# simonhmartin/genomics_general

Hardware: AMD Instinct MI355X
Metric: windows_per_sec (higher is better)
Workload: dtype u32 bit-planes / int32 counts / f64 statistics

## Files before the change

### genomics_general_amd/csrc/pg_pair2.hip

```cpp
#include "pg_internal.h"
#include "pg_pair_common.h"

#include <algorithm>
#include <cstdlib>
#include <cstring>

typedef __attribute__((address_space(4))) const uint32_t CU32;

__device__ __forceinline__ void store16(uint32_t *p, uint32_t a, uint32_t b, uint32_t c, uint32_t d) {
    *reinterpret_cast<uint4 *>(p) = make_uint4(a, b, c, d);
}

__device__ __forceinline__ void btrans4(uint32_t t0, uint32_t t1, uint32_t t2, uint32_t t3, uint32_t r[4]) {
    const uint32_t lo01 = __builtin_amdgcn_perm(t1, t0, 0x05010400u), hi01 = __builtin_amdgcn_perm(t1, t0, 0x07030602u);
    const uint32_t lo23 = __builtin_amdgcn_perm(t3, t2, 0x05010400u), hi23 = __builtin_amdgcn_perm(t3, t2, 0x07030602u);
    r[0] = __builtin_amdgcn_perm(lo23, lo01, 0x05040100u);
    r[1] = __builtin_amdgcn_perm(lo23, lo01, 0x07060302u);
    r[2] = __builtin_amdgcn_perm(hi23, hi01, 0x05040100u);
    r[3] = __builtin_amdgcn_perm(hi23, hi01, 0x07060302u);
}

struct RowOff { int v[16]; };

__device__ __forceinline__ RowOff make_row_off(int RS) {
    RowOff ro;
#pragma unroll
    for (int s = 0; s < 16; ++s) {
        int t = s * RS;
        asm volatile("" : "+s"(t));
        ro.v[s] = t;
    }
    return ro;
}

__device__ __forceinline__ void word_load(__amdgpu_buffer_rsrc_t rsrc, int b0, int RS, int row0, const RowOff &ro, uint32_t d[32]) {
    const int v0 = b0 + row0 * RS, v1 = v0 + 16 * RS;
#pragma unroll
    for (int s = 0; s < 16; ++s) d[s] = (uint32_t)__builtin_amdgcn_raw_buffer_load_b32(rsrc, v0, ro.v[s], 0);
#pragma unroll
    for (int s = 0; s < 16; ++s) d[16 + s] = (uint32_t)__builtin_amdgcn_raw_buffer_load_b32(rsrc, v1, ro.v[s], 0);
}

__device__ __forceinline__ void word_load16(__amdgpu_buffer_rsrc_t rsrc, int b0, int RS, int row0, const RowOff &ro, uint32_t d[32]) {
    const int v0 = b0 + row0 * RS, v1 = v0 + 16 * RS;
#pragma unroll
    for (int s = 0; s < 16; ++s) d[s] = (uint32_t)__builtin_amdgcn_raw_buffer_load_b16(rsrc, v0, ro.v[s], 0);
#pragma unroll
    for (int s = 0; s < 16; ++s) d[16 + s] = (uint32_t)__builtin_amdgcn_raw_buffer_load_b16(rsrc, v1, ro.v[s], 0);
}

__device__ __forceinline__ uint32_t merge16(uint32_t x0, uint32_t x1) { return pg_nib_expand4(x0) | (pg_nib_expand4(x1) << 4); }

__device__ __forceinline__ void word_called_presence(const uint32_t d[32], uint32_t v[4], uint32_t pa[4]) {
#pragma unroll
    for (int q = 0; q < 4; ++q) {
        const uint32_t *e = d + 8 * q;
        uint32_t r[4];
        btrans4(merge16(e[0], e[1]), merge16(e[2], e[3]), merge16(e[4], e[5]), merge16(e[6], e[7]), r);
        const uint32_t o = r[0] | r[1] | r[2] | r[3];
#pragma unroll
        for (int a = 0; a < 4; ++a) {
            const uint32_t piece = (a >= q ? (o >> (a - q)) : (o << (q - a))) & (0x11111111u << q);
            pa[a] = q ? (pa[a] | piece) : piece;
        }
#pragma unroll
        for (int k = 0; k < 4; ++k) {
            const uint32_t u = r[k] | (r[k] >> 1);
            const uint32_t c = (u | (u >> 2)) & 0x11111111u;
            v[k] = q ? (v[k] | (c << q)) : c;
        }
    }
}

__device__ __forceinline__ void poly_word(__amdgpu_buffer_rsrc_t rsrc, int h0, int RS, uint32_t vlist, const uint32_t SA[3],
                                          const uint32_t SE[2], uint32_t x[PG_XV_PLANES][4]) {
    uint32_t al[4][4];
#pragma unroll
    for (int q = 0; q < 4; ++q) {
        uint32_t d[8];
#pragma unroll
        for (int s = 0; s < 8; ++s) {
            const int row = __builtin_amdgcn_readlane((int)vlist, q * 8 + s) & 0xffff;
            d[s] = (uint32_t)__builtin_amdgcn_raw_buffer_load_b16(rsrc, h0 >> 1, row * RS, 0);
        }
        uint32_t r[4];
        btrans4(merge16(d[0], d[1]), merge16(d[2], d[3]), merge16(d[4], d[5]), merge16(d[6], d[7]), r);
#pragma unroll
        for (int k = 0; k < 4; ++k)
#pragma unroll
            for (int a = 0; a < 4; ++a) {
                const uint32_t piece = (a >= q ? (r[k] >> (a - q)) : (r[k] << (q - a))) & (0x11111111u << q);
                al[a][k] = q ? (al[a][k] | piece) : piece;
            }
    }
#pragma unroll
    for (int k = 0; k < 4; ++k) {
        const uint32_t ex = (al[0][k] & SE[0]) | (al[1][k] & SE[1]);
        x[0][k] = (al[0][k] & SA[0]) | (al[1][k] & SA[1]) | (al[2][k] & SA[2]);
        x[1][k] = (al[0][k] | al[1][k] | al[2][k] | al[3][k]) & ~ex;
    }
}

__device__ __forceinline__ void wave_or4(uint32_t v[4]) {
#define PG_DPP_OR4(ctrl, rmask)                                                                           \
    _Pragma("unroll") for (int i = 0; i < 4; ++i)                                                          \
        v[i] |= (uint32_t)__builtin_amdgcn_update_dpp(0, (int)v[i], ctrl, rmask, 0xf, false)
    PG_DPP_OR4(0x111, 0xf);
    PG_DPP_OR4(0x112, 0xf);
    PG_DPP_OR4(0x114, 0xf);
    PG_DPP_OR4(0x118, 0xf);
    PG_DPP_OR4(0x142, 0xa);
    PG_DPP_OR4(0x143, 0xc);
#undef PG_DPP_OR4
#pragma unroll
    for (int i = 0; i < 4; ++i) v[i] = (uint32_t)__builtin_amdgcn_readlane((int)v[i], 63);
}

__device__ __forceinline__ uint32_t poly_mask(const uint32_t p[4]) {
    return (p[0] & p[1]) | (p[2] & p[3]) | ((p[0] ^ p[1]) & (p[2] ^ p[3]));
}

__device__ __forceinline__ uint32_t tri_mask(const uint32_t p[4]) {
    return (p[0] & p[1] & (p[2] | p[3])) | (p[2] & p[3] & (p[0] | p[1]));
}
__device__ __forceinline__ uint32_t quad_mask(const uint32_t p[4]) { return p[0] & p[1] & p[2] & p[3]; }

__device__ __forceinline__ __amdgpu_buffer_rsrc_t group_rsrc(const int8_t *gt, int RS, int64_t first_row, int nrows) {
    return __builtin_amdgcn_make_buffer_rsrc(const_cast<int8_t *>(gt + first_row * (int64_t)RS), 0, nrows * RS, 0x00020000);
}

template <int NWAVE>
__device__ __forceinline__ bool xv_leader() { return (NWAVE == 1 ? threadIdx.x & 63 : threadIdx.x) == 0; }

struct XvWin {
    uint32_t *xv_base;
    int NP, h0, capw;
    int32_t *nwb, *mismatch;
    bool has_data;

    template <int NWAVE>
    __device__ __forceinline__ bool holds(int slot) const {
        if (slot >= capw) {
            if (xv_leader<NWAVE>()) atomicOr(mismatch, 2);
            return false;
        }
        return has_data;
    }
    __device__ __forceinline__ uint32_t *word(int slot) const { return xv_base + (size_t)slot * PG_XV_PLANES * (size_t)NP + 2 * h0; }
};

__device__ __forceinline__ XvWin make_xv_win(uint32_t *XV, const int64_t *goff, int b, int capg, int NP, int h0, int32_t *nw,
                                             int32_t *mismatch, bool has_data) {
    return {XV + (size_t)goff[b] * capg * PG_XV_PLANES * (size_t)NP, NP, h0, (int)(goff[b + 1] - goff[b]) * capg, &nw[b], mismatch, has_data};
}

template <int NWAVE>
__device__ __forceinline__ int xv_reserve(int32_t *nwb, int n, int *sh_slot) {
    if (NWAVE == 1) {
        int s0 = 0;
        if (xv_leader<1>()) s0 = atomicAdd(nwb, n);
        return __builtin_amdgcn_readfirstlane(s0);
    }
    if (xv_leader<NWAVE>()) *sh_slot = atomicAdd(nwb, n);
    __syncthreads();
    const int slot = __builtin_amdgcn_readfirstlane(*sh_slot);
    __syncthreads();
    return slot;
}

template <int NWAVE>
__device__ __forceinline__ void block_or4(uint32_t pr[4], uint32_t (*sh_pres)[NWAVE][4], int &parity, int lane) {
    wave_or4(pr);
    if (NWAVE > 1) {
        if (lane == 0) {
#pragma unroll
            for (int a = 0; a < 4; ++a) sh_pres[parity][threadIdx.x >> 6][a] = pr[a];
        }
        __syncthreads();
#pragma unroll
        for (int a = 0; a < 4; ++a) {
            uint32_t x = 0u;
#pragma unroll
            for (int wv = 0; wv < NWAVE; ++wv) x |= sh_pres[parity][wv][a];
            pr[a] = __builtin_amdgcn_readfirstlane(x);
        }
        parity ^= 1;
    }
}

__global__ __launch_bounds__(256) void k_presence(const int8_t *__restrict__ gt, int RS, const int64_t *__restrict__ win_lo,
                                                  const int64_t *__restrict__ win_hi, const int64_t *__restrict__ goff,
                                                  uint32_t *__restrict__ pres, int grp) {
    const int b = blockIdx.y, g = blockIdx.x;
    const int64_t lo = win_lo[b], hi = win_hi[b];
    const int W = (int)((hi - lo + 31) >> 5);
    const int w_begin = g * grp;
    if (w_begin >= W) return;
    const int w_end = (w_begin + grp < W) ? w_begin + grp : W;
    const int h0 = 4 * (blockIdx.z * 256 + threadIdx.x);
    const int64_t first = lo + 32ll * w_begin;
    const int nrows = (int)((hi - first) < 32ll * grp ? (hi - first) : 32ll * grp);
    const __amdgpu_buffer_rsrc_t rsrc = group_rsrc(gt, RS, first, nrows);
    uint32_t *dst = pres + (size_t)(goff[b] + g) * grp * 4u;
    const RowOff ro = make_row_off(RS);
    for (int w = w_begin; w < w_end; ++w) {
        uint32_t v[4], pa[4] = {0u, 0u, 0u, 0u};
        if (h0 < 2 * RS) {
            uint32_t d[32];
            word_load16(rsrc, h0 >> 1, RS, (w - w_begin) * 32, ro, d);
            word_called_presence(d, v, pa);
        }
        wave_or4(pa);
#pragma unroll
        for (int a = 0; a < 4; ++a)
            if ((threadIdx.x & 63) == 0 && pa[a]) atomicOr(&dst[(size_t)(w - w_begin) * 4u + a], pa[a]);
    }
}

__global__ __launch_bounds__(256) void k_word_scan(const int64_t *__restrict__ win_lo, const int64_t *__restrict__ win_hi,
                                                   const int64_t *__restrict__ goff, const uint32_t *__restrict__ pres,
                                                   int32_t *__restrict__ nw, int grp) {
    __shared__ int sh[256];
    __shared__ int carry;
    const int b = blockIdx.x, n_win = gridDim.x;
    const int64_t lo = win_lo[b], hi = win_hi[b];
    const int W = (int)((hi - lo + 31) >> 5);
    const int G = (W + grp - 1) / grp;
    if (threadIdx.x == 0) carry = 0;
    __syncthreads();
    for (int g0 = 0; g0 < G; g0 += 256) {
        const int g = g0 + threadIdx.x;
        int words = 0;
        if (g < G) {
            const int nwords = (W - g * grp < grp) ? W - g * grp : grp;
            const uint32_t *src = pres + (size_t)(goff[b] + g) * grp * 4u;
            int cnt = 0;
            for (int w = 0; w < nwords; ++w) {
                const uint32_t p[4] = {src[4 * w], src[4 * w + 1], src[4 * w + 2], src[4 * w + 3]};
                cnt += __builtin_popcount(poly_mask(p)) + __builtin_popcount(tri_mask(p)) + __builtin_popcount(quad_mask(p));
            }
            words = (cnt + 31) >> 5;
        }
        sh[threadIdx.x] = words;
        __syncthreads();
        for (int d = 1; d < 256; d <<= 1) {
            const int v = threadIdx.x >= d ? sh[threadIdx.x - d] : 0;
            __syncthreads();
            sh[threadIdx.x] += v;
            __syncthreads();
        }
        if (g < G) nw[n_win + goff[b] + g] = carry + sh[threadIdx.x] - words;
        __syncthreads();
        if (threadIdx.x == 255) carry += sh[255];
        __syncthreads();
    }
    if (threadIdx.x == 0) nw[b] = carry;
}

template <int TPB, int DIP, int PRES>
__global__ __launch_bounds__(TPB) void k_pack2(const int8_t *__restrict__ gt, int RS, const int64_t *__restrict__ win_lo,
                                               const int64_t *__restrict__ win_hi, const int64_t *__restrict__ goff,
                                               const int64_t *__restrict__ vgoff, uint32_t *__restrict__ Vp, int NPv,
                                               uint32_t *__restrict__ XV, int NP, int32_t *__restrict__ nw,
                                               int32_t *__restrict__ mismatch, const uint32_t *__restrict__ pres, int capg, int grp) {
    constexpr int NWAVE = TPB / 64;
    __shared__ uint32_t sh_pres[2][NWAVE][4];
    __shared__ uint4 sh_gp[PRES ? 1 : PG_GROUP_MAX];
    __shared__ int sh_slot;
    const int b = blockIdx.y, g = blockIdx.x, n_win = gridDim.y;
    const int64_t lo = win_lo[b], hi = win_hi[b];
    const int W = (int)((hi - lo + 31) >> 5);
    const int w_begin = g * grp;
    if (w_begin >= W) return;
    const int w_end = (w_begin + grp < W) ? w_begin + grp : W;
    const int t = blockIdx.z * TPB + threadIdx.x;
    const int lane = threadIdx.x & 63;
    const int h0 = 4 * t;
    const bool has_data = h0 < 2 * RS;
    const int u0 = DIP ? 2 * t : h0;
    const int64_t first = lo + 32ll * w_begin;
    const int nrows = (int)((hi - first) < 32ll * grp ? (hi - first) : 32ll * grp);
    const __amdgpu_buffer_rsrc_t rsrc = group_rsrc(gt, RS, first, nrows);
    uint32_t vlist = (uint32_t)nrows;
    int cnt = 0, nflush = 0, parity = 0;
    uint32_t bad = 0u;
    const XvWin xw = make_xv_win(XV, goff, b, capg, NP, h0, nw, mismatch, has_data);
    const uint32_t *pres_g = pres + (size_t)(goff[b] + g) * grp * 4u;
    const int64_t vg_base = vgoff[b] + (int64_t)(w_begin >> 2);
    const int gbase = PRES ? nw[n_win + goff[b] + g] : 0;
    auto flush = [&]() {
        const int slot = PRES ? gbase + nflush : xv_reserve<NWAVE>(xw.nwb, 1, &sh_slot);
        uint32_t A = 0u, E = 0u;
        {
            const int row = (int)(vlist & 0xffffu), ord = (int)(vlist >> 16);
            if (row < nrows) {
                const int wi = row >> 5, st = row & 31, bit = 4 * (st & 7) + (st >> 3);
                const uint4 pp = PRES ? *reinterpret_cast<const uint4 *>(pres_g + 4 * wi) : sh_gp[PRES ? 0 : wi];
                const uint32_t P = ((pp.x >> bit) & 1u) | (((pp.y >> bit) & 1u) << 1) | (((pp.z >> bit) & 1u) << 2) |
                                   (((pp.w >> bit) & 1u) << 3);
                const uint32_t A0 = P & (0u - P), P1 = P ^ A0, A1 = P1 & (0u - P1), P2 = P1 ^ A1, A2 = P2 & (0u - P2);
                A = ord == 0 ? A0 : (ord == 1 ? A1 : A2);
                E = (A - 1u) & P;
            }
        }
        const int src = (lane & 3) * 8 + ((lane >> 2) & 7);
        A = (uint32_t)__shfl((int)A, src, 64);
        E = (uint32_t)__shfl((int)E, src, 64);
        const uint32_t SA[3] = {(uint32_t)__builtin_amdgcn_ballot_w64(A == 1u), (uint32_t)__builtin_amdgcn_ballot_w64(A == 2u),
                                (uint32_t)__builtin_amdgcn_ballot_w64(A == 4u)};
        const uint32_t SE[2] = {(uint32_t)__builtin_amdgcn_ballot_w64((E & 1u) != 0u),
                                (uint32_t)__builtin_amdgcn_ballot_w64((E & 2u) != 0u)};
        if (xw.holds<NWAVE>(slot)) {
            uint32_t x[PG_XV_PLANES][4];
            poly_word(rsrc, h0, RS, vlist, SA, SE, x);
            uint32_t *o = xw.word(slot);
            store16(o, x[0][0], x[1][0], x[0][1], x[1][1]);
            store16(o + 4, x[0][2], x[1][2], x[0][3], x[1][3]);
        }
        ++nflush;
    };
    uint32_t dn[32];
#pragma unroll
    for (int s = 0; s < 32; ++s) dn[s] = 0u;
    const RowOff ro = make_row_off(RS);
    if (has_data) word_load16(rsrc, h0 >> 1, RS, 0, ro, dn);
    for (int wq = 0; 4 * wq + w_begin < w_end; ++wq) {
        uint32_t vhold[4][4];
#pragma unroll
        for (int k4 = 0; k4 < 4; ++k4) {
            const int w = w_begin + 4 * wq + k4;
            uint32_t v[4] = {0u, 0u, 0u, 0u}, pa[4] = {0u, 0u, 0u, 0u};
            const bool live = w < w_end;
            uint32_t d[32];
#pragma unroll
            for (int s = 0; s < 32; ++s) d[s] = dn[s];
            if (has_data) word_load16(rsrc, h0 >> 1, RS, (w + 1 - w_begin) * 32, ro, dn);
            if (live && has_data) word_called_presence(d, v, pa);
#pragma unroll
            for (int k = 0; k < 4; ++k) vhold[k][k4] = v[k];
            if (DIP) bad |= (v[0] ^ v[1]) | (v[2] ^ v[3]);
            if (live) {
                uint32_t pr[4];
                if (PRES) {
                    const uint32_t *src = pres + ((size_t)(goff[b] + g) * grp + (size_t)(w - w_begin)) * 4u;
#pragma unroll
                    for (int a = 0; a < 4; ++a) pr[a] = __builtin_amdgcn_readfirstlane(src[a]);
                } else {
#pragma unroll
                    for (int a = 0; a < 4; ++a) pr[a] = pa[a];
                    block_or4<NWAVE>(pr, sh_pres, parity, lane);
                }
                if (!PRES && threadIdx.x == 0) sh_gp[PRES ? 0 : w - w_begin] = make_uint4(pr[0], pr[1], pr[2], pr[3]);
                const int row_w = (w - w_begin) * 32;
                const uint32_t m3 = tri_mask(pr);
#pragma unroll 1
                for (int pass = 0; pass < 3; ++pass) {
                    uint32_t m = pass == 0 ? poly_mask(pr) : (pass == 1 ? m3 : quad_mask(pr));
                    if (pass && !m3) break;
                    const uint32_t tag = (uint32_t)pass << 16;
                    while (m) {
                        const int bit = __builtin_ctz(m);
                        m &= m - 1u;
                        vlist = lane == cnt ? ((uint32_t)(row_w + (bit & 3) * 8 + (bit >> 2)) | tag) : vlist;
                        ++cnt;
                    }
                    if (cnt >= 32) {
                        flush();
                        const uint32_t up = (uint32_t)__shfl((int)vlist, (lane + 32) & 63, 64);
                        vlist = lane < 32 ? up : (uint32_t)nrows;
                        cnt -= 32;
                    }
                }
            }
        }
        if (has_data) {
            if (DIP) {
                uint32_t *o = Vp + ((size_t)(vg_base + wq) * NPv + u0) * 4u;
                store16(o, vhold[0][0], vhold[0][1], vhold[0][2], vhold[0][3]);
                store16(o + 4, vhold[2][0], vhold[2][1], vhold[2][2], vhold[2][3]);
            } else {
                uint32_t *o = Vp + ((size_t)(vg_base + wq) * NPv + u0) * 4u;
#pragma unroll
                for (int k = 0; k < 4; ++k)
                    store16(o + 4 * k, vhold[k][0], vhold[k][1], vhold[k][2], vhold[k][3]);
            }
        }
    }
    if (cnt) flush();
    if (DIP && bad) atomicOr(mismatch, 1);
}

__device__ __forceinline__ uint32_t bfi_f0(uint32_t hi, uint32_t lo) { return (hi & 0xF0F0F0F0u) | (lo & 0x0F0F0F0Fu); }

__device__ __forceinline__ void trans_even(const uint32_t e[8], uint32_t r[4]) {
    btrans4(bfi_f0(e[1] << 4, e[0]), bfi_f0(e[3] << 4, e[2]), bfi_f0(e[5] << 4, e[4]), bfi_f0(e[7] << 4, e[6]), r);
}
__device__ __forceinline__ void trans_odd(const uint32_t e[8], uint32_t r[4]) {
    btrans4(bfi_f0(e[1], e[0] >> 4), bfi_f0(e[3], e[2] >> 4), bfi_f0(e[5], e[4] >> 4), bfi_f0(e[7], e[6] >> 4), r);
}
__device__ __forceinline__ void keep_presence(int q, const uint32_t re[4], const uint32_t ro[4], uint32_t Rq[8], uint32_t pa[4]) {
#pragma unroll
    for (int k = 0; k < 4; ++k) {
        Rq[2 * k] = re[k];
        Rq[2 * k + 1] = ro[k];
    }
    const uint32_t o = (re[0] | re[1] | re[2] | re[3]) | (ro[0] | ro[1] | ro[2] | ro[3]);
#pragma unroll
    for (int a = 0; a < 4; ++a) {
        const uint32_t piece = (a >= q ? (o >> (a - q)) : (o << (q - a))) & (0x11111111u << q);
        pa[a] = q ? (pa[a] | piece) : piece;
    }
}

__device__ __forceinline__ void word_called_presence_keep(const uint32_t d[32], uint32_t v[8], uint32_t pa[4], uint32_t R[4][8]) {
#pragma unroll
    for (int q = 0; q < 4; ++q) {
        uint32_t re[4], ro[4];
        trans_even(d + 8 * q, re);
        trans_odd(d + 8 * q, ro);
        keep_presence(q, re, ro, R[q], pa);
#pragma unroll
        for (int k = 0; k < 8; ++k) {
            const uint32_t t = R[q][k] + 0x77777777u;
            const uint32_t c = (q == 3 ? t : (t >> (3 - q))) & (0x11111111u << q);
            v[k] = q ? (v[k] | c) : c;
        }
    }
}

template <int NWAVE, bool STAGED>
struct XvSink {
    XvWin win;
    int *sh_slot;
    uint4 *cell;
    int stride, burst;
    int nxs;

    __device__ __forceinline__ XvSink(const XvWin &w, int *sh_slot_, uint4 *cell_, int stride_, int burst_)
        : win(w), sh_slot(sh_slot_), cell(cell_), stride(stride_), burst(burst_), nxs(0) {}
    __device__ __forceinline__ void flush() {
        if (!nxs) return;
        const int slot0 = xv_reserve<NWAVE>(win.nwb, nxs, sh_slot);
        for (int k = 0; k < nxs; ++k)
            if (win.template holds<NWAVE>(slot0 + k)) {
                uint4 *o = reinterpret_cast<uint4 *>(win.word(slot0 + k));
#pragma unroll
                for (int i = 0; i < 4; ++i) o[i] = cell[(4 * k + i) * stride];
            }
        nxs = 0;
    }
    __device__ __forceinline__ void put(const uint32_t xo[8], const uint32_t vo[8]) {
        if (STAGED) {
            if (win.has_data) {
#pragma unroll
                for (int i = 0; i < 4; ++i) cell[(4 * nxs + i) * stride] = make_uint4(xo[2 * i], vo[2 * i], xo[2 * i + 1], vo[2 * i + 1]);
            }
            if (++nxs == burst) flush();
        } else {
            const int slot = xv_reserve<NWAVE>(win.nwb, 1, sh_slot);
            if (win.template holds<NWAVE>(slot)) {
                uint32_t *o = win.word(slot);
#pragma unroll
                for (int i = 0; i < 4; ++i) store16(o + 4 * i, xo[2 * i], vo[2 * i], xo[2 * i + 1], vo[2 * i + 1]);
            }
        }
    }
};

__device__ __forceinline__ uint32_t nz_nibbles(uint32_t x) { return ((x + 0x77777777u) >> 3) & 0x11111111u; }


template <class Sink>
struct VsCompactor {
    uint32_t cur[8], xo[8], vo[8];
    int cnt;
    uint32_t MA, ME;
    Sink &out;

    __device__ __forceinline__ explicit VsCompactor(Sink &s) : cnt(0), MA(0u), ME(0u), out(s) {
#pragma unroll
        for (int k = 0; k < 8; ++k) cur[k] = xo[k] = vo[k] = 0u;
    }
    __device__ __forceinline__ void finish_dword(int qd) {
        const uint32_t nME = ~ME;
#pragma unroll
        for (int k = 0; k < 8; ++k) {
            xo[k] |= nz_nibbles(cur[k] & MA) << qd;
            vo[k] |= nz_nibbles(cur[k] & nME) << qd;
            cur[k] = 0u;
        }
        MA = 0u;
        ME = 0u;
    }
    __device__ __forceinline__ void store_word() {
        out.put(xo, vo);
#pragma unroll
        for (int k = 0; k < 8; ++k) xo[k] = vo[k] = 0u;
    }
    __device__ __forceinline__ void append(const uint32_t (&Rq)[8], int j, uint32_t A, uint32_t E) {
        const int sh = 4 * (cnt & 7);
#pragma unroll
        for (int k = 0; k < 8; ++k) cur[k] |= __builtin_amdgcn_ubfe(Rq[k], 4 * j, 4) << sh;
        MA |= A << sh;
        ME |= E << sh;
        ++cnt;
        if ((cnt & 7) == 0) {
            finish_dword((cnt >> 3) - 1);
            if (cnt == 32) {
                store_word();
                cnt = 0;
            }
        }
    }
    __device__ __forceinline__ void finish() {
        if (cnt & 7) finish_dword(cnt >> 3);
        if (cnt) store_word();
    }
};

template <class Sink>
__device__ __forceinline__ void emit_poly_sites(const uint32_t pr[4], const uint32_t (&R)[4][8], VsCompactor<Sink> &vs, int lane) {
    const uint32_t m0 = poly_mask(pr);
    if (m0) {
        const int lb = lane & 31;
        const uint32_t Pl = __builtin_amdgcn_ubfe(pr[0], lb, 1) | (__builtin_amdgcn_ubfe(pr[1], lb, 1) << 1) |
                            (__builtin_amdgcn_ubfe(pr[2], lb, 1) << 2) | (__builtin_amdgcn_ubfe(pr[3], lb, 1) << 3);
        const uint32_t A0l = Pl & (0u - Pl);
#pragma unroll
        for (int q = 0; q < 4; ++q) {
            uint32_t mq = m0 & (0x11111111u << q);
            while (mq) {
                const int bit = __builtin_ctz(mq);
                mq &= mq - 1u;
                vs.append(R[q], bit >> 2, (uint32_t)__builtin_amdgcn_readlane((int)A0l, bit), 0u);
            }
        }
        const uint32_t m3 = tri_mask(pr);
        if (m3) {
#pragma unroll 1
            for (int pass = 1; pass < 3; ++pass) {
                uint32_t m = pass == 1 ? m3 : quad_mask(pr);
                while (m) {
                    const int bit = __builtin_ctz(m);
                    m &= m - 1u;
                    const uint32_t P = (uint32_t)__builtin_amdgcn_readlane((int)Pl, bit);
                    const uint32_t A0 = P & (0u - P), P1 = P ^ A0, A1 = P1 & (0u - P1), P2 = P1 ^ A1, A2 = P2 & (0u - P2);
                    const uint32_t A = pass == 1 ? A1 : A2;
                    const int q = bit & 3;
                    if (q == 0) vs.append(R[0], bit >> 2, A, (A - 1u) & P);
                    else if (q == 1) vs.append(R[1], bit >> 2, A, (A - 1u) & P);
                    else if (q == 2) vs.append(R[2], bit >> 2, A, (A - 1u) & P);
                    else vs.append(R[3], bit >> 2, A, (A - 1u) & P);
                }
            }
        }
    }
}

constexpr int PACK_FUSE_XC = 2;
constexpr int PACK_FUSE_NB = 3;
constexpr int PACK_FUSE_SPINS = 1 << 22;

__device__ __forceinline__ void fuse_frags(const uint4 *fb, int s, int UW, const int ia[4], const int ib[2], v8i fa_[4], v8i fb_[2]) {
#pragma unroll
    for (int p = 0; p < 4; ++p) {
        const uint4 x = fb[2 * s * UW + ia[p]];
        fa_[p][0] = (int)x.x; fa_[p][1] = (int)x.y; fa_[p][2] = (int)x.z; fa_[p][3] = (int)x.w;
    }
#pragma unroll
    for (int p = 0; p < 2; ++p) {
        const uint4 x = fb[2 * s * UW + ib[p]];
        fb_[p][0] = (int)x.x; fb_[p][1] = (int)x.y; fb_[p][2] = (int)x.z; fb_[p][3] = (int)x.w;
    }
}

template <int DIP>
__device__ __forceinline__ void pack3_fused(const int8_t *__restrict__ gt, int RS, const int64_t *__restrict__ win_lo,
                                            const int64_t *__restrict__ win_hi, const int64_t *__restrict__ goff,
                                            uint32_t *__restrict__ XV, int NP, int32_t *__restrict__ nw,
                                            int32_t *__restrict__ mismatch, int capg, const PgFuseArgs &fa) {
    constexpr int VN = DIP ? 4 : 8;
    extern __shared__ uint4 fz_lds[];
    int b, kp;
    if (!pg_deal_window(blockIdx.x, fa.kparts, fa.n_win, b, kp)) return;
    const int UW = 32 * fa.T;
    const int lane = threadIdx.x & 63, wave = __builtin_amdgcn_readfirstlane(threadIdx.x >> 6);
    uint4 *const frag = fz_lds;
    uint4 *const stage_x = fz_lds + PACK_FUSE_NB * 8 * UW + wave * (PACK_FUSE_XC * 4 * 64);
    int *const ready = reinterpret_cast<int *>(fz_lds + PACK_FUSE_NB * 8 * UW + 8 * (PACK_FUSE_XC * 4 * 64)), *const done = ready + PACK_FUSE_NB;
    const int64_t lo = win_lo[b], hi = win_hi[b];
    const int W = (int)((hi - lo + 31) >> 5);
    const int w_begin = (int)((long long)W * kp / fa.kparts), w_end = (int)((long long)W * (kp + 1) / fa.kparts);
    const int nit = (w_end - w_begin + 7) >> 3;
    const int h0 = 8 * lane;
    const bool has_data = h0 < 2 * RS;
    const int u0 = VN * lane;
    uint32_t bad = 0u;
    typedef XvSink<1, true> Sink;
    Sink xs(make_xv_win(XV, goff, b, capg, NP, h0, nw, mismatch, has_data), nullptr,  stage_x + lane,  64,
             PACK_FUSE_XC);
    VsCompactor<Sink> vs(xs);
    auto word_rsrc = [&](int w) -> __amdgpu_buffer_rsrc_t {
        const int64_t row = lo + 32ll * w;
        const int n = w < w_end ? (int)((hi - row) < 32 ? (hi - row) : 32) : 0;
        return group_rsrc(gt, RS, n ? row : lo, n);
    };
    const int r = lane & 31, kb = lane >> 5;
    int ia[4], ib[2];
#pragma unroll
    for (int p = 0; p < 4; ++p) ia[p] = kb * UW + 32 * (int)fa.a[wave][p] + r;
#pragma unroll
    for (int p = 0; p < 2; ++p) ib[p] = kb * UW + 32 * (int)fa.b[wave][p] + r;
    v16f acc[4];
#pragma unroll
    for (int p = 0; p < 4; ++p)
#pragma unroll
        for (int e = 0; e < 16; ++e) acc[p][e] = 0.0f;
    if (threadIdx.x < 2 * PACK_FUSE_NB) ready[threadIdx.x] = threadIdx.x == 2 * PACK_FUSE_NB - 1 ? -8 : 0;
    for (int i = threadIdx.x; i < 8 * UW; i += 512) frag[(PACK_FUSE_NB - 1) * 8 * UW + i] = make_uint4(0u, 0u, 0u, 0u);
    bool stalled = false;
    auto wait_ge = [&](int *ctr, int target) {
        for (int spins = 0; __builtin_amdgcn_readfirstlane(__hip_atomic_load(ctr, __ATOMIC_ACQUIRE, __HIP_MEMORY_SCOPE_WORKGROUP)) < target;) {
            __builtin_amdgcn_s_sleep(1);
            if (++spins > PACK_FUSE_SPINS) { stalled = true; break; }
        }
    };
    auto arrive = [&](int *ctr) {
        if (lane == 0) __hip_atomic_fetch_add(ctr, 1, __ATOMIC_RELEASE, __HIP_MEMORY_SCOPE_WORKGROUP);
    };
    uint32_t dn[32];
#pragma unroll
    for (int s = 0; s < 32; ++s) dn[s] = 0u;
    const RowOff ro = make_row_off(RS);
    const int lane_off = has_data ? 4 * lane : 0x40000000;
    word_load(word_rsrc(w_begin + wave), lane_off, RS, 0, ro, dn);
    __syncthreads();
    int slot = 0, round8 = 0, pslot = PACK_FUSE_NB - 1, pround8 = -8;
    for (int it = 0; it < nit; ++it) {
        const int w = w_begin + 8 * it + wave;
        uint32_t pa[4] = {0u, 0u, 0u, 0u};
        uint32_t R[4][8];
        const bool live = w < w_end;
        uint32_t d[32];
#pragma unroll
        for (int s = 0; s < 32; ++s) d[s] = dn[s];
        word_load(word_rsrc(w + 8), lane_off, RS, 0, ro, dn);
        wait_ge(&ready[pslot], pround8 + 8);
        const uint4 *fb = frag + pslot * 8 * UW;
#pragma unroll
        for (int q = 0; q < 4; ++q) {
            v8i fa_[4], fb_[2];
            fuse_frags(fb, q, UW, ia, ib, fa_, fb_);
            uint32_t re[4], rq[4];
            __builtin_amdgcn_sched_barrier(0);
            trans_even(d + 8 * q, re);
            asm volatile("" : "+v"(re[0]), "+v"(re[1]), "+v"(re[2]), "+v"(re[3]));
            __builtin_amdgcn_sched_barrier(0);
            acc[0] = pg_mfma_fp4(fa_[0], fb_[0], acc[0]);
            __builtin_amdgcn_sched_barrier(0);
            trans_odd(d + 8 * q, rq);
            asm volatile("" : "+v"(rq[0]), "+v"(rq[1]), "+v"(rq[2]), "+v"(rq[3]));
            __builtin_amdgcn_sched_barrier(0);
            acc[1] = pg_mfma_fp4(fa_[1], fb_[1], acc[1]);
            __builtin_amdgcn_sched_barrier(0);
            keep_presence(q, re, rq, R[q], pa);
            asm volatile("" : "+v"(pa[0]), "+v"(pa[1]), "+v"(pa[2]), "+v"(pa[3]));
            __builtin_amdgcn_sched_barrier(0);
            acc[2] = pg_mfma_fp4(fa_[2], fb_[0], acc[2]);
            acc[3] = pg_mfma_fp4(fa_[3], fb_[1], acc[3]);
            __builtin_amdgcn_sched_barrier(0);
        }
        arrive(&done[pslot]);
        wait_ge(&done[slot], round8);
        {
            uint4 *cell = frag + (slot * 8 + wave) * UW + u0;
#pragma unroll
            for (int k = 0; k < VN; ++k) {
                const int hk = DIP ? 2 * k : k;
                uint32_t c[4];
#pragma unroll
                for (int q = 0; q < 4; ++q) {
                    const uint32_t t = R[q][hk] + 0x77777777u;
                    if (DIP) bad |= t ^ (R[q][hk + 1] + 0x77777777u);
                    c[q] = (t >> 3) & 0x11111111u;
                }
                if (u0 + k < UW) cell[k] = make_uint4(c[0], c[1], c[2], c[3]);
            }
        }
        arrive(&ready[slot]);
        if (live) {
            uint32_t pr[4];
#pragma unroll
            for (int a = 0; a < 4; ++a) pr[a] = pa[a];
            wave_or4(pr);
            emit_poly_sites(pr, R, vs, lane);
        }
        pslot = slot;
        pround8 = round8;
        if (++slot == PACK_FUSE_NB) { slot = 0; round8 += 8; }
    }
    wait_ge(&ready[pslot], pround8 + 8);
#pragma unroll
    for (int q = 0; q < 4; ++q) {
        v8i fa_[4], fb_[2];
        fuse_frags(frag + pslot * 8 * UW, q, UW, ia, ib, fa_, fb_);
#pragma unroll
        for (int p = 0; p < 4; ++p) acc[p] = pg_mfma_fp4(fa_[p], fb_[p & 1], acc[p]);
    }
    if (stalled && lane == 0) atomicOr(mismatch, PG_FLAG_FUSE_STALL);
    vs.finish();
    xs.flush();
    if (DIP && (bad & 0x88888888u)) atomicOr(mismatch, 1);
    const int n = fa.n_units;
    int32_t *Cw = fa.Cmat + (size_t)b * n * n;
#pragma unroll
    for (int p = 0; p < 4; ++p)
        if ((fa.mask[wave] >> p) & 1) pg_store_tile<4>(acc[p], fa.a[wave][p], fa.b[wave][p & 1], lane, n, fa.diag, fa.kparts > 1, Cw);
}

constexpr int PACK_CELLS = 24;
template <int TPB, int DIP, int BURST, int FUSE>
__global__ __launch_bounds__(TPB) void k_pack3(const int8_t *__restrict__ gt, int RS, const int64_t *__restrict__ win_lo,
                                               const int64_t *__restrict__ win_hi, const int64_t *__restrict__ goff,
                                               const int64_t *__restrict__ vgoff, uint32_t *__restrict__ Vp, int NPv,
                                               uint32_t *__restrict__ XV, int NP, int32_t *__restrict__ nw,
                                               int32_t *__restrict__ mismatch, int capg, int grp, int fq, int perm, PgFuseArgs fa) {
    if constexpr (FUSE) {
        pack3_fused<DIP>(gt, RS, win_lo, win_hi, goff, XV, NP, nw, mismatch, capg, fa);
        return;
    }
    constexpr int NWAVE = TPB / 64;
    constexpr int VN = DIP ? 4 : 8;
    const int FQ = fq, xc = (PACK_CELLS - fq * VN) / 4;
    __shared__ uint32_t sh_pres[2][NWAVE][4];
    __shared__ int sh_slot;
    __shared__ uint4 stage[BURST ? PACK_CELLS * TPB : 1];
    uint4 *const stage_v = stage, *const stage_x = stage + FQ * VN * TPB;
    int nq = 0, wq_first = 0;
    const int b = (int)(((unsigned long long)blockIdx.y * (unsigned)perm) % gridDim.y), g = blockIdx.x;
    const int64_t lo = win_lo[b], hi = win_hi[b];
    const int W = (int)((hi - lo + 31) >> 5);
    const int w_begin = g * grp;
    if (w_begin >= W) return;
    const int w_end = (w_begin + grp < W) ? w_begin + grp : W;
    const int t = threadIdx.x;
    const int lane = threadIdx.x & 63;
    const int h0 = 8 * t;
    const bool has_data = h0 < 2 * RS;
    const int u0 = DIP ? 4 * t : h0;
    const int64_t first = lo + 32ll * w_begin;
    const int nrows = (int)((hi - first) < 32ll * grp ? (hi - first) : 32ll * grp);
    const __amdgpu_buffer_rsrc_t rsrc = group_rsrc(gt, RS, first, nrows);
    int parity = 0;
    uint32_t bad = 0u;
    const int64_t vg_base = vgoff[b] + (int64_t)(w_begin >> 2);
    typedef XvSink<NWAVE, BURST != 0> Sink;
    Sink xs(make_xv_win(XV, goff, b, capg, NP, h0, nw, mismatch, has_data), &sh_slot,  stage_x + t,  TPB,
             xc);
    VsCompactor<Sink> vs(xs);
    auto flush_v = [&]() {
        if (has_data)
            for (int q = 0; q < nq; ++q) {
                uint4 *o = reinterpret_cast<uint4 *>(Vp + ((size_t)(vg_base + wq_first + q) * NPv + u0) * 4u);
#pragma unroll
                for (int k = 0; k < VN; ++k) o[k] = stage_v[(q * VN + k) * TPB + t];
            }
        nq = 0;
    };
    uint32_t dn[32];
#pragma unroll
    for (int s = 0; s < 32; ++s) dn[s] = 0u;
    const RowOff ro = make_row_off(RS);
    if (has_data) word_load(rsrc, 4 * t, RS, 0, ro, dn);
    for (int wq = 0; 4 * wq + w_begin < w_end; ++wq) {
        uint32_t vhold[8][4];
#pragma unroll
        for (int k4 = 0; k4 < 4; ++k4) {
            const int w = w_begin + 4 * wq + k4;
            uint32_t v[8] = {0u, 0u, 0u, 0u, 0u, 0u, 0u, 0u}, pa[4] = {0u, 0u, 0u, 0u};
            uint32_t R[4][8];
#pragma unroll
            for (int q = 0; q < 4; ++q)
#pragma unroll
                for (int k = 0; k < 8; ++k) R[q][k] = 0u;
            const bool live = w < w_end;
            uint32_t d[32];
#pragma unroll
            for (int s = 0; s < 32; ++s) d[s] = dn[s];
            if (has_data) word_load(rsrc, 4 * t, RS, (w + 1 - w_begin) * 32, ro, dn);
            if (live && has_data) word_called_presence_keep(d, v, pa, R);
#pragma unroll
            for (int k = 0; k < 8; ++k) vhold[k][k4] = v[k];
            if (DIP) bad |= (v[0] ^ v[1]) | (v[2] ^ v[3]) | (v[4] ^ v[5]) | (v[6] ^ v[7]);
            if (live) {
                uint32_t pr[4];
#pragma unroll
                for (int a = 0; a < 4; ++a) pr[a] = pa[a];
                block_or4<NWAVE>(pr, sh_pres, parity, lane);
                emit_poly_sites(pr, R, vs, lane);
            }
        }
        if (BURST) {
            if (nq == 0) wq_first = wq;
            if (has_data) {
#pragma unroll
                for (int k = 0; k < VN; ++k) {
                    const int hk = DIP ? 2 * k : k;
                    stage_v[(nq * VN + k) * TPB + t] = make_uint4(vhold[hk][0], vhold[hk][1], vhold[hk][2], vhold[hk][3]);
                }
            }
            if (++nq == FQ) flush_v();
        } else if (has_data) {
            uint32_t *o = Vp + ((size_t)(vg_base + wq) * NPv + u0) * 4u;
#pragma unroll
            for (int k = 0; k < VN; ++k) {
                const int hk = DIP ? 2 * k : k;
                store16(o + 4 * k, vhold[hk][0], vhold[hk][1], vhold[hk][2], vhold[hk][3]);
            }
        }
    }
    vs.finish();
    if (BURST) {
        flush_v();
        xs.flush();
    }
    if (DIP && bad) atomicOr(mismatch, 1);
}

template <int DIP>
static void launch_pack2(hipStream_t st, int threads, dim3 grid, const int8_t *gt, int RS, const int64_t *win_lo,
                         const int64_t *win_hi, const int64_t *goff, const int64_t *vgoff, uint32_t *Vp, int NPv, uint32_t *XV,
                         int NP, int32_t *nw, int32_t *mismatch, uint32_t *pres, int capg, int grp, PgPackRoute route,
                         const PgPairSwitches &sw) {
    if (route == PG_PACK_3) {
        const int lanes = (threads + 1) / 2;
#define PG_PACK3B(T, B) hipLaunchKernelGGL((k_pack3<T, DIP, B, 0>), grid, dim3(T), 0, st, gt, RS, win_lo, win_hi, goff, vgoff, Vp, NPv, XV, NP, nw, mismatch, capg, grp, fq, perm, PgFuseArgs())
#define PG_PACK3(T) PG_PACK3B(T, 0)
        const int fq = DIP ? 4 : 2;
        const int perm = pg_pack_perm(sw, (int)grid.y);
        const bool burst = pg_pack3_burst(NP, sw);
        if (lanes <= 64 && burst) PG_PACK3B(64, 1);
        else if (burst) PG_PACK3B(128, 1);
        else if (lanes <= 64) PG_PACK3(64);
        else if (lanes <= 128) PG_PACK3(128);
        else if (lanes <= 256) PG_PACK3(256);
        else PG_PACK3(512);
#undef PG_PACK3
#undef PG_PACK3B
        return;
    }
    if (threads <= 64)
        hipLaunchKernelGGL((k_pack2<64, DIP, 0>), grid, dim3(64), 0, st, gt, RS, win_lo, win_hi, goff, vgoff, Vp, NPv, XV, NP, nw, mismatch, pres, capg, grp);
    else if (threads <= 128)
        hipLaunchKernelGGL((k_pack2<128, DIP, 0>), grid, dim3(128), 0, st, gt, RS, win_lo, win_hi, goff, vgoff, Vp, NPv, XV, NP, nw, mismatch, pres, capg, grp);
    else if (route == PG_PACK_2)
        hipLaunchKernelGGL((k_pack2<256, DIP, 0>), grid, dim3(256), 0, st, gt, RS, win_lo, win_hi, goff, vgoff, Vp, NPv, XV, NP, nw, mismatch, pres, capg, grp);
    else {
        grid.z = (threads + 255) / 256;
        hipLaunchKernelGGL(k_presence, grid, dim3(256), 0, st, gt, RS, win_lo, win_hi, goff, pres, grp);
        hipLaunchKernelGGL(k_word_scan, dim3(grid.y), dim3(256), 0, st, win_lo, win_hi, goff, pres, nw, grp);
        hipLaunchKernelGGL((k_pack2<256, DIP, 1>), grid, dim3(256), 0, st, gt, RS, win_lo, win_hi, goff, vgoff, Vp, NPv, XV, NP, nw, mismatch, pres, capg, grp);
    }
}

int pg_launch_pack_fused(hipStream_t st, const int8_t *gt, int RS, const int64_t *win_lo, const int64_t *win_hi, const int64_t *goff,
                         int n_win, int64_t max_words, int64_t avg_words, uint32_t *XV, int NP, int32_t *nw, int dip, int32_t *mismatch,
                         int capg, int n_units, int32_t *Cmat) {
    if (n_win <= 0) return 0;
    PgFuseArgs fa;
    fa.n_win = n_win;
    fa.n_units = n_units;
    fa.T = (n_units + 31) / 32;
    fa.diag = dip ? 1 : 0;
    fa.Cmat = Cmat;
    pg_fuse_tasks(fa.T, fa);
    int64_t kparts = n_win >= 1024 ? 1 : (1024 + n_win - 1) / n_win;
    kparts = std::min<int64_t>(kparts, std::max<int64_t>(1, avg_words / 64));
    kparts = std::max<int64_t>(kparts, pg_exact_parts(max_words * 32));
    fa.kparts = (int)kparts;
    pg_zero_if_parts(st, Cmat, n_win, n_units, kparts);
    const size_t lds = (size_t)(PACK_FUSE_NB * 8 * 32 * fa.T + 8 * PACK_FUSE_XC * 4 * 64 + 2) * sizeof(uint4);
    const int64_t blocks = pg_deal_blocks(n_win, kparts);
#define PG_PACK3F(D)                                                                                                              \
    do {                                                                                                                          \
        static bool ready = false;                                   \
        if (!ready) {                                                                                                             \
            if (hipFuncSetAttribute(reinterpret_cast<const void *>(&k_pack3<512, D, 0, 1>), hipFuncAttributeMaxDynamicSharedMemorySize, \
                                    (PACK_FUSE_NB * 8 * 32 * 7 + 8 * PACK_FUSE_XC * 4 * 64 + 2) * (int)sizeof(uint4)) != hipSuccess) return 1; \
            ready = true;                                                                                                         \
        }                                                                                                                         \
        hipLaunchKernelGGL((k_pack3<512, D, 0, 1>), dim3((unsigned)blocks), dim3(512), lds, st, gt, RS, win_lo, win_hi, goff,         \
                           (const int64_t *)nullptr, (uint32_t *)nullptr, 0, XV, NP, nw, mismatch, capg, 0, 0, 1, fa);           \
    } while (0)
    if (dip) PG_PACK3F(1);
    else PG_PACK3F(0);
#undef PG_PACK3F
    return 0;
}

void pg_launch_pack2(hipStream_t st, const int8_t *gt, int RS, const int64_t *win_lo, const int64_t *win_hi,
                     const int64_t *goff, const int64_t *vgoff, int n_win, int max_groups, int64_t total_groups, uint32_t *Vp,
                     int NPv, uint32_t *XV, int NP, int32_t *nw, int dip, int32_t *mismatch, uint32_t *pres, int capg, int grp,
                     PgPackRoute route, const PgPairSwitches &sw) {
    if (n_win <= 0 || max_groups <= 0) return;
    const int threads = NP / 4;
    if (route == PG_PACK_2_PRESENCE) (void)hipMemsetAsync(pres, 0, (size_t)total_groups * grp * 16u, st);
    dim3 grid(max_groups, n_win);
    if (dip) launch_pack2<1>(st, threads, grid, gt, RS, win_lo, win_hi, goff, vgoff, Vp, NPv, XV, NP, nw, mismatch, pres, capg, grp, route, sw);
    else launch_pack2<0>(st, threads, grid, gt, RS, win_lo, win_hi, goff, vgoff, Vp, NPv, XV, NP, nw, mismatch, pres, capg, grp, route, sw);
}

struct PairCtx {
    int win, row0, nsub, col0, lower, lane, ks;
};

__device__ __forceinline__ bool pair_decode(const PgTask2 *__restrict__ tasks, int n_tasks, int kso, int n_win, PairCtx &c) {
    int rem;
    if (!pg_deal_window(blockIdx.x, n_tasks * kso, n_win, c.win, rem)) return false;
    const int wave = __builtin_amdgcn_readfirstlane(threadIdx.x >> 6);
    c.ks = (rem / n_tasks) * 4 + wave;
    c.lane = threadIdx.x & 63;
    const PgTask2 tk = tasks[rem % n_tasks];
    c.row0 = __builtin_amdgcn_readfirstlane(tk.row0);
    c.nsub = __builtin_amdgcn_readfirstlane(tk.nsub);
    c.col0 = __builtin_amdgcn_readfirstlane(tk.col0);
    c.lower = __builtin_amdgcn_readfirstlane(tk.lower);
    return true;
}

template <int R>
__device__ __forceinline__ bool block_reduce(uint32_t (&acc)[R], uint32_t (*red)[64], int lane) {
    const int wave = __builtin_amdgcn_readfirstlane(threadIdx.x >> 6);
    if (wave) {
#pragma unroll
        for (int r = 0; r < R; ++r) red[(wave - 1) * R + r][lane] = acc[r];
    }
    __syncthreads();
    if (wave) return false;
#pragma unroll
    for (int r = 0; r < R; ++r) acc[r] += red[r][lane] + red[R + r][lane] + red[2 * R + r][lane];
    return true;
}

template <int R>
__device__ __forceinline__ void pair_store_circ(const uint32_t (&acc)[R], int row0, int col0, int lane, int nvalid, int n, int diag,
                                                int atomic, int32_t *__restrict__ M) {
    if (lane >= nvalid) return;
    int j = col0 + lane;
    if (j >= n) j -= n;
    const int h = n >> 1;
#pragma unroll
    for (int r = 0; r < R; ++r) {
        const int i = row0 + r;
        if (i >= n) continue;
        int d = j - i;
        if (d < 0) d += n;
        const bool keep = d == 0 ? (diag != 0) : (d <= h && !(2 * d == n && i > j));
        if (!keep) continue;
        int32_t *dst = i <= j ? &M[(size_t)i * n + j] : &M[(size_t)j * n + i];
        if (atomic) { if (acc[r]) atomicAdd(dst, (int32_t)acc[r]); }
        else *dst = (int32_t)acc[r];
    }
}

__device__ __forceinline__ uint32_t bcnt_acc(uint32_t x, uint32_t acc) {
    uint32_t r;
    asm("v_bcnt_u32_b32 %0, %1, %2" : "=v"(r) : "v"(x), "v"(acc));
    return r;
}

#include "pg_pairc_loop.inc"

__device__ __forceinline__ void pairC_body(const uint32_t *__restrict__ Vp, int64_t vg0, int nwq, int NPv, const PairCtx &c,
                                           uint32_t (&acc)[8], int n_units) {
    int j = c.col0 + c.lane;
    if (j >= n_units) j -= n_units;
    const uint32_t stride = (uint32_t)NPv * 16u;
    const int chunk = (int)(0x7fffffffu / stride) > 2 ? (int)(0x7fffffffu / stride) - 2 : 1;
    for (int q0 = 0; q0 < nwq; q0 += chunk) {
        const int nq = (nwq - q0 < chunk) ? nwq - q0 : chunk;
        const uint32_t *base = Vp + (size_t)(vg0 + q0) * NPv * 4u;
        const uint64_t b64 = (uint64_t)base;
        const uint64_t ubase = ((uint64_t)(uint32_t)__builtin_amdgcn_readfirstlane((int)(b64 >> 32)) << 32) |
                               (uint32_t)__builtin_amdgcn_readfirstlane((int)(uint32_t)b64);
        uint32_t soff = (uint32_t)c.row0 * 16u, voff = (uint32_t)j * 16u;
        uint32_t n6 = (uint32_t)__builtin_amdgcn_readfirstlane(nq / 6), rem = (uint32_t)__builtin_amdgcn_readfirstlane(nq % 6);
        asm volatile(PG_PAIRC_LOOP_ASM
                     : "+v"(acc[0]), "+v"(acc[1]), "+v"(acc[2]), "+v"(acc[3]), "+v"(acc[4]), "+v"(acc[5]), "+v"(acc[6]),
                       "+v"(acc[7]), "+s"(soff), "+v"(voff), "+s"(n6)
                     : "s"(ubase), "s"(stride), "s"(rem)
                     : PG_PAIRC_LOOP_CLOBBERS);
    }
}

__global__ __launch_bounds__(256) void k_pairC(const uint32_t *__restrict__ Vp, const int64_t *__restrict__ vgoff, int n_win,
                                               const PgTask2 *__restrict__ tasks, int n_tasks, int kso, int NPv, int n_units,
                                               int diag, int32_t *__restrict__ Cmat) {
    __shared__ uint32_t red[3 * 8][64];
    PairCtx c;
    if (!pair_decode(tasks, n_tasks, kso, n_win, c)) return;
    const int64_t vg_all = vgoff[c.win];
    const int nwq_all = (int)(vgoff[c.win + 1] - vg_all);
    const int parts = 4 * kso;
    const int q0 = (int)((long long)nwq_all * c.ks / parts), q1 = (int)((long long)nwq_all * (c.ks + 1) / parts);
    uint32_t acc[8];
#pragma unroll
    for (int r = 0; r < 8; ++r) acc[r] = 0u;
    if (q1 > q0) pairC_body(Vp, vg_all + q0, q1 - q0, NPv, c, acc, n_units);
    if (block_reduce<8>(acc, red, c.lane)) {
        int32_t *Cw = Cmat + (size_t)c.win * n_units * n_units;
        pair_store_circ<8>(acc, c.row0, c.col0, c.lane, c.nsub, n_units, diag, kso > 1, Cw);
    }
}

static int pick_kso(int n_win, int n_tasks, int64_t steps_per_window, int min_steps) {
    int64_t waves = (int64_t)n_win * n_tasks * 4;
    int ks = 1;
    while (ks < 16 && waves * ks < 8192 && steps_per_window / (ks * 8) >= min_steps) ks *= 2;
    return ks;
}

void pg_launch_pairC(hipStream_t st, const uint32_t *Vp, const int64_t *vgoff, int n_win, const PgTask2 *tasks, int n_tasks,
                     int NPv, int n_units, int diag, int64_t avg_wq, int32_t *Cmat) {
    if (n_win <= 0 || n_tasks <= 0) return;
    const int kso = pick_kso(n_win, n_tasks, avg_wq, 24);
    pg_zero_if_parts(st, Cmat, n_win, n_units, kso);
    const int64_t blocks = pg_deal_blocks(n_win, (int64_t)n_tasks * kso);
    hipLaunchKernelGGL(k_pairC, dim3((unsigned)blocks), dim3(256), 0, st, Vp, vgoff, n_win, tasks, n_tasks, kso, NPv, n_units,
                       diag, Cmat);
}

#include "pg_paird_loop.inc"

__device__ __forceinline__ void pairD_body(const uint32_t *__restrict__ XVw, int w0, int w1, int NP, int N, const PairCtx &c,
                                           uint32_t (&acc)[16]) {
    int j = c.col0 + c.lane;
    if (j >= N) j -= N;
    const uint32_t stride = (uint32_t)NP * 4u * PG_XV_PLANES;
    const int chunk = (int)(0x7fffffffu / stride) > 2 ? (int)(0x7fffffffu / stride) - 2 : 1;
    for (int q0 = w0; q0 < w1; q0 += chunk) {
        const int nq = (w1 - q0 < chunk) ? w1 - q0 : chunk;
        const uint32_t *base = XVw + (size_t)q0 * NP * PG_XV_PLANES;
        const uint64_t b64 = (uint64_t)base;
        const uint64_t ubase = ((uint64_t)(uint32_t)__builtin_amdgcn_readfirstlane((int)(b64 >> 32)) << 32) |
                               (uint32_t)__builtin_amdgcn_readfirstlane((int)(uint32_t)b64);
        uint32_t soff = (uint32_t)c.row0 * 8u, voff = (uint32_t)j * 8u;
        uint32_t n6 = (uint32_t)__builtin_amdgcn_readfirstlane(nq / 6), rem = (uint32_t)__builtin_amdgcn_readfirstlane(nq % 6);
        asm volatile(PG_PAIRD_LOOP_ASM
                     : "+v"(acc[0]), "+v"(acc[1]), "+v"(acc[2]), "+v"(acc[3]), "+v"(acc[4]), "+v"(acc[5]), "+v"(acc[6]),
                       "+v"(acc[7]), "+v"(acc[8]), "+v"(acc[9]), "+v"(acc[10]), "+v"(acc[11]), "+v"(acc[12]), "+v"(acc[13]),
                       "+v"(acc[14]), "+v"(acc[15]), "+s"(soff), "+v"(voff), "+s"(n6)
                     : "s"(ubase), "s"(stride), "s"(rem)
                     : PG_PAIRD_LOOP_CLOBBERS);
    }
}

__global__ __launch_bounds__(256) void k_pairD(const uint32_t *__restrict__ XV, const int32_t *__restrict__ nw,
                                               const int64_t *__restrict__ goff, int n_win, const PgTask2 *__restrict__ tasks,
                                               int n_tasks, int kso, int NP, int N, int32_t *__restrict__ Dmat, int capg) {
    __shared__ uint32_t red[3 * 16][64];
    PairCtx c;
    if (!pair_decode(tasks, n_tasks, kso, n_win, c)) return;
    const uint32_t *XVw = XV + (size_t)goff[c.win] * capg * PG_XV_PLANES * (size_t)NP;
    const int capw = (int)(goff[c.win + 1] - goff[c.win]) * capg;
    const int n_all = __builtin_amdgcn_readfirstlane(nw[c.win]);
    const int n_words = n_all < capw ? n_all : capw;
    const int parts = 4 * kso;
    const int a = (int)((long long)n_words * c.ks / parts), b = (int)((long long)n_words * (c.ks + 1) / parts);
    int32_t *Dw = Dmat + (size_t)c.win * N * N;
    uint32_t acc[16];
#pragma unroll
    for (int r = 0; r < 16; ++r) acc[r] = 0u;
    if (b > a) pairD_body(XVw, a, b, NP, N, c, acc);
    if (block_reduce<16>(acc, red, c.lane)) pair_store_circ<16>(acc, c.row0, c.col0, c.lane, c.nsub, N, 0, kso > 1, Dw);
}

void pg_launch_pairD(hipStream_t st, const uint32_t *XV, const int32_t *nw, const int64_t *goff, int n_win,
                     const PgTask2 *tasks, int n_tasks, int NP, int N, int64_t avg_groups, int32_t *Dmat, int capg) {
    if (n_win <= 0 || n_tasks <= 0) return;
    const int kso = pick_kso(n_win, n_tasks, avg_groups, 1);
    pg_zero_if_parts(st, Dmat, n_win, N, kso);
    const int64_t blocks = pg_deal_blocks(n_win, (int64_t)n_tasks * kso);
    hipLaunchKernelGGL(k_pairD, dim3((unsigned)blocks), dim3(256), 0, st, XV, nw, goff, n_win, tasks, n_tasks, kso, NP, N, Dmat, capg);
}

__global__ __launch_bounds__(256) void k_expand(const int32_t *__restrict__ Cmat, const int32_t *__restrict__ Dmat, int N, int cN,
                                                int cshift, int32_t *__restrict__ Cfull, int32_t *__restrict__ Dfull) {
    const int32_t *Cw = Cmat + (size_t)blockIdx.y * cN * cN;
    const int32_t *Dw = Dmat + (size_t)blockIdx.y * N * N;
    int32_t *Co = Cfull + (size_t)blockIdx.y * N * N;
    int32_t *Do = Dfull + (size_t)blockIdx.y * N * N;
    for (int idx = blockIdx.x * blockDim.x + threadIdx.x; idx < N * N; idx += gridDim.x * blockDim.x) {
        const int i = idx / N, j = idx - i * N;
        if (i == j) { Co[idx] = 0; Do[idx] = 0; continue; }
        const int a = i < j ? i : j, b = i < j ? j : i;
        Co[idx] = Cw[(size_t)(a >> cshift) * cN + (b >> cshift)];
        Do[idx] = Dw[(size_t)a * N + b];
    }
}

void pg_launch_expand(hipStream_t st, const int32_t *Cmat, const int32_t *Dmat, int N, int cN, int cshift, int n_win,
                      int32_t *Cfull, int32_t *Dfull) {
    if (n_win <= 0) return;
    int bx = (N * N + 255) / 256;
    if (bx > 64) bx = 64;
    hipLaunchKernelGGL(k_expand, dim3(bx, n_win), dim3(256), 0, st, Cmat, Dmat, N, cN, cshift, Cfull, Dfull);
}
```

Baseline: 351,000.

## Stream next-word loads piecewise into the consumed register buffer

Replaces the double-buffered dn/d prefetch with a single d buffer. Each quarter of the next word is loaded into d right after that quarter has been transposed, and the loads sit between the MFMA calls. The per-iteration buffer resource is now built by advancing a base pointer and row count instead of recomputing from the window index. This cuts VGPR pressure by dropping the 32-register copy and the second buffer, at the risk of load latency being exposed when d is used in the next iteration. The rows_left clamp also changes how tail and dead waves compute their zero-length resources.

Result: no change. 353,800, median of 6 (+0.8%).

```diff
diff --git a/genomics_general_amd/csrc/pg_pair2.hip b/genomics_general_amd/csrc/pg_pair2.hip
--- a/genomics_general_amd/csrc/pg_pair2.hip
+++ b/genomics_general_amd/csrc/pg_pair2.hip
@@ -33,12 +33,14 @@
     return ro;
 }
 
+__device__ __forceinline__ void piece_load(__amdgpu_buffer_rsrc_t rsrc, int b0, int RS, int row0, const RowOff &ro, int q, uint32_t e[8]) {
+    const int v = b0 + (row0 + 16 * (q >> 1)) * RS;
+#pragma unroll
+    for (int s = 0; s < 8; ++s) e[s] = (uint32_t)__builtin_amdgcn_raw_buffer_load_b32(rsrc, v, ro.v[8 * (q & 1) + s], 0);
+}
 __device__ __forceinline__ void word_load(__amdgpu_buffer_rsrc_t rsrc, int b0, int RS, int row0, const RowOff &ro, uint32_t d[32]) {
-    const int v0 = b0 + row0 * RS, v1 = v0 + 16 * RS;
-#pragma unroll
-    for (int s = 0; s < 16; ++s) d[s] = (uint32_t)__builtin_amdgcn_raw_buffer_load_b32(rsrc, v0, ro.v[s], 0);
-#pragma unroll
-    for (int s = 0; s < 16; ++s) d[16 + s] = (uint32_t)__builtin_amdgcn_raw_buffer_load_b32(rsrc, v1, ro.v[s], 0);
+#pragma unroll
+    for (int q = 0; q < 4; ++q) piece_load(rsrc, b0, RS, row0, ro, q, d + 8 * q);
 }
 
 __device__ __forceinline__ void word_load16(__amdgpu_buffer_rsrc_t rsrc, int b0, int RS, int row0, const RowOff &ro, uint32_t d[32]) {
@@ -125,8 +127,11 @@
 }
 __device__ __forceinline__ uint32_t quad_mask(const uint32_t p[4]) { return p[0] & p[1] & p[2] & p[3]; }
 
+__device__ __forceinline__ __amdgpu_buffer_rsrc_t rows_rsrc(const int8_t *first, int RS, int nrows) {
+    return __builtin_amdgcn_make_buffer_rsrc(const_cast<int8_t *>(first), 0, nrows * RS, 0x00020000);
+}
 __device__ __forceinline__ __amdgpu_buffer_rsrc_t group_rsrc(const int8_t *gt, int RS, int64_t first_row, int nrows) {
-    return __builtin_amdgcn_make_buffer_rsrc(const_cast<int8_t *>(gt + first_row * (int64_t)RS), 0, nrows * RS, 0x00020000);
+    return rows_rsrc(gt + first_row * (int64_t)RS, RS, nrows);
 }
 
 template <int NWAVE>
@@ -600,10 +605,17 @@
     Sink xs(make_xv_win(XV, goff, b, capg, NP, h0, nw, mismatch, has_data), nullptr,  stage_x + lane,  64,
              PACK_FUSE_XC);
     VsCompactor<Sink> vs(xs);
-    auto word_rsrc = [&](int w) -> __amdgpu_buffer_rsrc_t {
-        const int64_t row = lo + 32ll * w;
-        const int n = w < w_end ? (int)((hi - row) < 32 ? (hi - row) : 32) : 0;
-        return group_rsrc(gt, RS, n ? row : lo, n);
+    const int64_t row_first = lo + 32ll * (w_begin + wave), row_end = 32ll * w_end < hi - lo ? lo + 32ll * w_end : hi;
+    const int8_t *word_base = gt + row_first * (int64_t)RS;
+    int rows_left = (int)(row_end - row_first);
+    auto next_word_rsrc = [&]() -> __amdgpu_buffer_rsrc_t {
+        int n = rows_left < 32 ? rows_left : 32;
+        asm volatile("" : "+s"(n));
+        n = n < 0 ? 0 : n;
+        const __amdgpu_buffer_rsrc_t rsrc = rows_rsrc(word_base, RS, n);
+        word_base += 256ll * RS;
+        rows_left -= 256;
+        return rsrc;
     };
     const int r = lane & 31, kb = lane >> 5;
     int ia[4], ib[2];
@@ -628,12 +640,10 @@
     auto arrive = [&](int *ctr) {
         if (lane == 0) __hip_atomic_fetch_add(ctr, 1, __ATOMIC_RELEASE, __HIP_MEMORY_SCOPE_WORKGROUP);
     };
-    uint32_t dn[32];
-#pragma unroll
-    for (int s = 0; s < 32; ++s) dn[s] = 0u;
+    uint32_t d[32];
     const RowOff ro = make_row_off(RS);
     const int lane_off = has_data ? 4 * lane : 0x40000000;
-    word_load(word_rsrc(w_begin + wave), lane_off, RS, 0, ro, dn);
+    word_load(next_word_rsrc(), lane_off, RS, 0, ro, d);
     __syncthreads();
     int slot = 0, round8 = 0, pslot = PACK_FUSE_NB - 1, pround8 = -8;
     for (int it = 0; it < nit; ++it) {
@@ -641,10 +651,7 @@
         uint32_t pa[4] = {0u, 0u, 0u, 0u};
         uint32_t R[4][8];
         const bool live = w < w_end;
-        uint32_t d[32];
-#pragma unroll
-        for (int s = 0; s < 32; ++s) d[s] = dn[s];
-        word_load(word_rsrc(w + 8), lane_off, RS, 0, ro, dn);
+        const __amdgpu_buffer_rsrc_t rsrc_next = next_word_rsrc();
         wait_ge(&ready[pslot], pround8 + 8);
         const uint4 *fb = frag + pslot * 8 * UW;
 #pragma unroll
@@ -660,6 +667,8 @@
             __builtin_amdgcn_sched_barrier(0);
             trans_odd(d + 8 * q, rq);
             asm volatile("" : "+v"(rq[0]), "+v"(rq[1]), "+v"(rq[2]), "+v"(rq[3]));
+            __builtin_amdgcn_sched_barrier(0);
+            piece_load(rsrc_next, lane_off, RS, 0, ro, q, d + 8 * q);
             __builtin_amdgcn_sched_barrier(0);
             acc[1] = pg_mfma_fp4(fa_[1], fb_[1], acc[1]);
             __builtin_amdgcn_sched_barrier(0);
```
